# naver/deep-image-retrieval

Measured on AMD Instinct MI355X. Metric: images/sec descriptor extraction (resnet101-GeM, 1024x1024), higher is better.
Workload: dtype fp16p

## Files before the change

### deep-image-retrieval_amd/csrc/c_api.hip

```cpp
#include <new>

#include "engine.h"
#include "pointwise.h"

namespace dir {
const char* last_error();
}
using namespace dir;

static constexpr int kSimSplitMinRows = 32768;

#define DIR_TRY try {
#define DIR_CATCH                                                   \
    }                                                               \
    catch (const std::bad_alloc&) {                                 \
        return fail(DIR_ERR_NOMEM, "out of host memory");           \
    }                                                               \
    catch (const std::exception& ex) {                              \
        return fail(DIR_ERR_INVALID, std::string("exception: ") + ex.what()); \
    }                                                               \
    catch (...) {                                                   \
        return fail(DIR_ERR_INVALID, "unknown exception");          \
    }

// ... 405 lines not shown

static int fill_conv_args(ConvArgs& a, const void* x, const void* w, const float* bias,
                          const void* res, void* y, int B, int H, int W, int Cin, int Cout, int R,
                          int S, int stride, int pad, int OH, int OW, int relu) {
    if (!x || !w || !bias || !y) return fail(DIR_ERR_INVALID, "conv: null pointer");
    if (B <= 0 || H <= 0 || W <= 0 || Cin <= 0 || Cout <= 0 || R <= 0 || S <= 0 || stride <= 0 ||
        pad < 0 || OH <= 0 || OW <= 0)
        return fail(DIR_ERR_INVALID, "conv: bad dimension");
    memset(&a, 0, sizeof(a));
    a.x = (const uint16_t*)x;
    a.w = (const uint16_t*)w;
    a.bias = bias;
    a.res = (const uint16_t*)res;
    a.y = (uint16_t*)y;
    a.B = B; a.H = H; a.W = W; a.Cin = Cin; a.OH = OH; a.OW = OW; a.Cout = Cout;
    a.R = R; a.S = S; a.stride = stride; a.pad = pad; a.relu = relu ? 1 : 0;
    a.M = B * OH * OW;
    a.Ktot = R * S * Cin;
    a.T = a.Ktot / 64;
    return DIR_OK;
}

int dir_conv_bn_act(const void* x, const void* w, const float* bias, const void* res, void* y,
                    int B, int H, int W, int Cin, int Cout, int R, int S, int stride, int pad,
                    int OH, int OW, int relu, int dtype, int variant, void* stream) {
    DIR_TRY
    ConvArgs a;
    int rc = fill_conv_args(a, x, w, bias, res, y, B, H, W, Cin, Cout, R, S, stride, pad, OH, OW, relu);
    if (rc != DIR_OK) return rc;
    return conv_launch(a, dtype, variant, (hipStream_t)stream);
    DIR_CATCH
}

int dir_conv_bn_act_splitk(const void* x, const void* w, const float* bias, const void* res, void* y,
                           int B, int H, int W, int Cin, int Cout, int R, int S, int stride, int pad,
                           int OH, int OW, int relu, int dtype, int variant, int ksplit, void* scratch,
                           size_t scratch_bytes, int* ksplit_used, void* stream) {
    DIR_TRY
    ConvArgs a;
    int rc = fill_conv_args(a, x, w, bias, res, y, B, H, W, Cin, Cout, R, S, stride, pad, OH, OW, relu);
    if (rc != DIR_OK) return rc;
    if (variant < 0) variant = conv_pick_variant(a);
    a.ksplit = ksplit < 0 ? conv_splitk_factor(variant, a) : ksplit;
    a.partial = (float*)scratch;
    if (a.ksplit > 1 && conv_splitk_bytes(a, a.ksplit) > scratch_bytes)
        return fail(DIR_ERR_WORKSPACE, "conv: split-K scratch too small");
    if (ksplit_used) *ksplit_used = a.ksplit > 1 ? a.ksplit : 1;
    return conv_launch(a, dtype, variant, (hipStream_t)stream);
    DIR_CATCH
}

int dir_conv_c3c1(const void* t2, const void* w3, const float* bias3, const void* res, void* y, const void* w1,
                  const float* bias1, void* t1, int B, int H, int W, int P, int P2, int relu3, int relu1, int dtype,
                  void* stream) {
    DIR_TRY
    ConvArgs a;
    int rc = fill_conv_args(a, t2, w3, bias3, res, y, B, H, W, P, 4 * P, 1, 1, 1, 0, H, W, relu3);
    if (rc != DIR_OK) return rc;
    if (!w1 || !bias1 || !t1 || !res) return fail(DIR_ERR_INVALID, "conv_c3c1: null pointer");
    if (dtype != DIR_BF16 && dtype != DIR_FP16) return fail(DIR_ERR_INVALID, "conv_c3c1: bad dtype");
    a.w2 = (const uint16_t*)w1;
    a.bias2 = bias1;
    a.y2 = (uint16_t*)t1;
    a.Cout2 = P2;
    a.relu2 = relu1 ? 1 : 0;
    if (!conv_c3c1_admissible(a))
// ... 344 lines not shown
```

### deep-image-retrieval_amd/csrc/conv_patchw.hip

```cpp
#include "dir_common.h"
#include "conv_igemm.h"

#ifndef DIR_PATCHW_ABL
#define DIR_PATCHW_ABL 0
#endif

namespace dir {

static constexpr uint32_t kOOBw = 0x80000000u;

__device__ __forceinline__ void dma16w(__amdgpu_buffer_rsrc_t rsrc, char* lds, uint32_t voff, int soff) {
    __builtin_amdgcn_raw_ptr_buffer_load_lds(rsrc, (DIR_LDS void*)lds, 16, voff, soff, 0, 0);
}

template <class DT>
__global__ void __launch_bounds__(512) conv_patch3x3w_kernel(const ConvArgs a) {
    constexpr int TH = 16, TW = 32, PH = TH + 2, PW = TW + 2, PP = PH * PW;
    constexpr int NTH = 512, BN = 128;
    constexpr int NPL = (PP * 4 + NTH - 1) / NTH;
    constexpr int PLANE_BYTES = NPL * NTH * 16;
    constexpr int TN = 4, TMR = 2;
    constexpr int WSTAGE = 3 * BN * 64, NBW = WSTAGE / (NTH * 16);
    constexpr int NBW_X = (DIR_PATCHW_ABL & 16) ? 2 : 0;
    constexpr int NPL_X = (DIR_PATCHW_ABL & 32) ? 7 : 0;
    constexpr int NSTW = 3;
    constexpr int WOFF = 2 * PLANE_BYTES;
    constexpr int EROW = TN * 128 + 16;
    typedef typename DT::frag_t frag_t;
    static_assert(WOFF + NSTW * WSTAGE <= 160 * 1024 && NBW * NTH * 16 == WSTAGE, "LDS map");

    extern __shared__ __attribute__((aligned(16))) char smem[];

// ... 378 lines not shown
            const f32x4_t f1 = *(const f32x4_t*)(ebase + mrow * EROW + ecol * 4 + 16);
            const int ox = ox0 + mrow;
            if (oy < a.OH && ox < a.OW) {
                float v[8] = {f0[0], f0[1], f0[2], f0[3], f1[0], f1[1], f1[2], f1[3]};
                const size_t o = ((size_t)(b * a.OH + oy) * a.OW + ox) * a.Cout + ncol;
                if (a.res) {
                    const u32x4_t rv = gload16(a.res + o);
#pragma unroll
                    for (int e = 0; e < 4; ++e) {
                        float lo, hi;
                        DT::unpack(rv[e], lo, hi);
                        v[2 * e] += lo;
                        v[2 * e + 1] += hi;
                    }
                }
                if (a.relu) {
#pragma unroll
                    for (int e = 0; e < 8; ++e) v[e] = fmaxf(v[e], 0.f);
                }
                u32x4_t ov;
#pragma unroll
                for (int e = 0; e < 4; ++e) ov[e] = DT::pack(v[2 * e], v[2 * e + 1]);
                gstore16(a.y + o, ov);
                ovf.see(ov);
            }
        }
        __builtin_amdgcn_fence(__ATOMIC_RELEASE, "wavefront");
        __builtin_amdgcn_wave_barrier();
        __builtin_amdgcn_fence(__ATOMIC_ACQUIRE, "wavefront");
    }
    ovf.flush(a.ovf);
}

bool conv_patch3x3w_admissible(const ConvArgs& a) {
    return a.R == 3 && a.S == 3 && a.stride == 1 && a.pad == 1 && a.H == a.OH && a.W == a.OW && a.Cin % 32 == 0 &&
           a.Cin >= 64 && a.Cout % 128 == 0 && (size_t)a.B * a.H * a.W * a.Cin * 2 < (1ull << 31) &&
           (size_t)a.Cout * a.Ktot * 2 < (1ull << 31);
}

__global__ void __launch_bounds__(256) pack_patchw_kernel(const uint16_t* w, uint16_t* out, int Cout, int Cin) {
    const int NQ = Cin / 32;
    const long pieces = (long)Cout * 9 * Cin / 8;
    for (long i = (long)blockIdx.x * 256 + threadIdx.x; i < pieces; i += (long)gridDim.x * 256) {
        const int L = (int)(i % 1536);
        long t = i / 1536;
        const int r = (int)(t % 3);
        t /= 3;
        const int q = (int)(t % NQ);
        const int tn = (int)(t / NQ);
        const int s = L >> 9, n = (L & 511) >> 2, pos = L & 3;
        const size_t src = ((size_t)((tn * 128 + n) * 9 + r * 3 + s)) * Cin + q * 32 + ((pos ^ ((n >> 2) & 3)) << 3);
        gstore16(out + i * 8, gload16(w + src));
    }
}

hipError_t conv_patch3x3w_pack(const uint16_t* w, uint16_t* out, int Cout, int Cin, hipStream_t stream) {
    const long pieces = (long)Cout * 9 * Cin / 8;
    const int grid = (int)((pieces + 255) / 256 < 1024 ? (pieces + 255) / 256 : 1024);
    hipLaunchKernelGGL(pack_patchw_kernel, dim3(grid), dim3(256), 0, stream, w, out, Cout, Cin);
    return hipGetLastError();
}

template <class DT>
static hipError_t launch_patch_w(const ConvArgs& a, hipStream_t stream) {
    constexpr int LDS = 2 * 5 * 512 * 16 + 3 * 3 * 128 * 64;
    static_assert(LDS <= 160 * 1024 && LDS >= 8 * 32 * (4 * 128 + 16), "LDS map (the staging area aliases it)");
    ConvArgs b = a;
    b.x_bytes = (uint32_t)((size_t)a.B * a.H * a.W * a.Cin * 2);
    b.w_bytes = (uint32_t)((size_t)a.Cout * a.Ktot * 2);
    const long blocks = (long)a.B * ((a.OH + 15) / 16) * ((a.OW + 31) / 32) * (a.Cout / 128);
    if (!env().no_patchw_lc) {
        void* scratch = nullptr;
        if (!b.w_pw && env().patchw_pack) {
            if (hipError_t e = hipMallocAsync(&scratch, b.w_bytes, stream); e != hipSuccess) return e;
            if (hipError_t e = conv_patch3x3w_pack(a.w, (uint16_t*)scratch, a.Cout, a.Cin, stream); e != hipSuccess) {
                (void)hipFreeAsync(scratch, stream);
                return e;
            }
            b.w_pw = (const uint16_t*)scratch;
        }
        auto kern = conv_patch3x3w_lc_kernel<DT>;
        static std::atomic<uint64_t> attr_lc{0};
        if (hipError_t e = ensure_dynamic_lds((const void*)kern, LDS, attr_lc); e != hipSuccess) return e;
        hipLaunchKernelGGL(kern, dim3((unsigned)blocks), dim3(768), LDS, stream, b);
        hipError_t e = hipGetLastError();
        if (scratch) {
            const hipError_t f = hipFreeAsync(scratch, stream);
            if (e == hipSuccess) e = f;
        }
        return e;
    }
    auto kern = conv_patch3x3w_kernel<DT>;
    static std::atomic<uint64_t> attr_done{0};
    if (hipError_t e = ensure_dynamic_lds((const void*)kern, LDS, attr_done); e != hipSuccess) return e;
    hipLaunchKernelGGL(kern, dim3((unsigned)blocks), dim3(512), LDS, stream, b);
    return hipGetLastError();
}

hipError_t conv_patch3x3w_launch(const ConvArgs& a, int dtype, hipStream_t stream) {
    return dtype == DIR_BF16 ? launch_patch_w<BF16>(a, stream) : launch_patch_w<FP16>(a, stream);
}

}
```

### deep-image-retrieval_amd/csrc/dir_common.h

```cpp
#pragma once
#include <hip/hip_runtime.h>
#include <stdint.h>
#include <string.h>
#include <atomic>
#include <string>

#include "../../include/dir_engine.h"

namespace dir {

typedef __attribute__((ext_vector_type(8))) __bf16 bf16x8_t;
typedef __attribute__((ext_vector_type(8))) _Float16 f16x8_t;
typedef __attribute__((ext_vector_type(16))) float f32x16_t;
typedef __attribute__((ext_vector_type(4))) float f32x4_t;
typedef __attribute__((ext_vector_type(4))) uint32_t u32x4_t;
typedef __attribute__((ext_vector_type(2))) uint32_t u32x2_t;
typedef __attribute__((ext_vector_type(2))) float f32x2_t;
typedef __attribute__((ext_vector_type(2))) __bf16 bf16x2_t;
typedef __attribute__((ext_vector_type(2))) _Float16 f16x2_t;

#define DIR_GLOBAL __attribute__((address_space(1)))
#define DIR_LDS __attribute__((address_space(3)))

void set_error(const std::string& msg);
int fail(int code, const std::string& msg);

#define DIR_HIP_CHECK(expr)                                                                \
    do {                                                                                   \
        hipError_t _e = (expr);                                                            \
        if (_e != hipSuccess)                                                              \
            return ::dir::fail(DIR_ERR_HIP, std::string(#expr) + ": " + hipGetErrorString(_e)); \
    } while (0)

struct Env {
    bool c3c1_off = false, c3c1_force = false;
    bool no_ds_seam = false, no_dual = false;
    bool rev_conv1 = false, rev_conv3 = false;
    bool unfused_stem = false, stem_v1 = false;
    bool no_patchlc = false, no_wreg = false, no_patchw = false, no_x3 = false, no_patchs = false;
    bool patchw_pack = false, no_patchw_pack = false;
    bool small_k2 = false;
    bool no_patchs2 = false;
    bool x3_k2048 = false;
    bool lc1x1 = false;
    bool no_c3c1lc = false;
    bool no_smallmap = false;
    bool no_wregd = false;
    bool no_patchw_lc = false;
    bool no_xcdmap = false;
    bool no_pair_patch = false, pair_acts = false;
    int pair_stages = 1;
    bool sim_v1 = false, sim_exact = false;
    bool experiments = false;
    bool no_inplace = false;
    bool no_stem_u8 = false;
    bool stem_pair_old = false;
    bool stem_u8_prep = false;
    bool stem_u8_wg8 = false;
    int stem_u8_seg = 0;
};
const Env& env();
void reload_env();

__host__ __device__ inline uint16_t f32_to_bf16_bits(float f) {
    uint32_t u;
    memcpy(&u, &f, 4);
    if ((u & 0x7fffffffu) > 0x7f800000u) return (uint16_t)((u >> 16) | 0x40);
    u += 0x7fffu + ((u >> 16) & 1u);
    return (uint16_t)(u >> 16);
}
__host__ __device__ inline float bf16_bits_to_f32(uint16_t h) {
    uint32_t u = ((uint32_t)h) << 16;
    float f;
    memcpy(&f, &u, 4);
    return f;
}
__host__ __device__ inline uint16_t f32_to_f16_bits(float f) {
    _Float16 h = (_Float16)f;
    uint16_t b;
    memcpy(&b, &h, 2);
    return b;
// ... 128 lines not shown
```

### deep-image-retrieval_amd/csrc/engine.hip

```cpp
#include "engine.h"

#include <math.h>
#include <algorithm>

namespace dir {

static thread_local std::string g_err;
void set_error(const std::string& msg) { g_err = msg; }
int fail(int code, const std::string& msg) {
    g_err = msg;
    return code;
}
const char* last_error() { return g_err.c_str(); }


static Env read_env() {
    Env e;
    auto on = [](const char* k) { return getenv(k) != nullptr; };
    const char* mode = getenv("DIRTORCH_AMD_C3C1");
    e.c3c1_off = mode && mode[0] == '0';
    e.c3c1_force = mode && mode[0] == 'f';
    e.no_ds_seam = on("DIRTORCH_AMD_NO_DS_SEAM");
    e.no_dual = on("DIRTORCH_AMD_NO_DUAL");
    e.rev_conv1 = on("DIRTORCH_AMD_REV_CONV1");
    e.rev_conv3 = on("DIRTORCH_AMD_REV_CONV3");
    e.unfused_stem = on("DIRTORCH_AMD_UNFUSED_STEM");
    e.stem_v1 = on("DIRTORCH_AMD_STEM_V1");
    e.no_patchlc = on("DIRTORCH_AMD_NO_PATCHLC");
    e.no_wreg = on("DIRTORCH_AMD_NO_WREG");
    e.no_wregd = on("DIRTORCH_AMD_NO_WREGD");
    e.no_smallmap = on("DIRTORCH_AMD_NO_SMALLMAP");
    e.no_c3c1lc = on("DIRTORCH_AMD_NO_C3C1LC");
    e.lc1x1 = on("DIRTORCH_AMD_LC1X1");
    e.x3_k2048 = on("DIRTORCH_AMD_X3_K2048");
    e.no_patchs2 = on("DIRTORCH_AMD_NO_PATCHS2");
    e.small_k2 = on("DIRTORCH_AMD_SMALL_K2");
    e.patchw_pack = on("DIRTORCH_AMD_PATCHW_PACK");
    e.no_patchw_pack = on("DIRTORCH_AMD_NO_PATCHW_PACK");
    e.no_patchw = on("DIRTORCH_AMD_NO_PATCHW");
    e.no_x3 = on("DIRTORCH_AMD_NO_X3");
    e.no_patchs = on("DIRTORCH_AMD_NO_PATCHS");
    e.no_patchw_lc = on("DIRTORCH_AMD_NO_PATCHW_LC");
    e.no_xcdmap = on("DIRTORCH_AMD_NO_XCDMAP");
    e.no_pair_patch = on("DIRTORCH_AMD_NO_PAIR_PATCH");
    e.pair_acts = on("DIRTORCH_AMD_PAIR_ACTS");
    if (const char* s = getenv("DIRTORCH_AMD_PAIR_STAGES")) e.pair_stages = atoi(s);
    e.sim_v1 = on("DIRTORCH_AMD_SIM_V1");
    e.sim_exact = on("DIRTORCH_AMD_SIM_EXACT");
    e.experiments = on("DIRTORCH_AMD_EXPERIMENTS");
    e.no_inplace = on("DIRTORCH_AMD_NO_INPLACE");
    e.no_stem_u8 = on("DIRTORCH_AMD_NO_STEM_U8");
    e.stem_u8_wg8 = on("DIRTORCH_AMD_STEM_U8_WG8");
    e.stem_u8_prep = on("DIRTORCH_AMD_STEM_U8_PREP");
    e.stem_pair_old = on("DIRTORCH_AMD_STEM_PAIR_OLD");
    if (const char* s = getenv("DIRTORCH_AMD_STEM_U8_SEG")) e.stem_u8_seg = atoi(s);
    return e;
}
static Env g_env[2];
static std::atomic<int> g_env_cur{-1};
static std::atomic_flag g_env_lock = ATOMIC_FLAG_INIT;
static void publish_env() {
    while (g_env_lock.test_and_set(std::memory_order_acquire)) {
    }
    const int cur = g_env_cur.load(std::memory_order_relaxed);
    const int nxt = cur < 0 ? 0 : 1 - cur;
    g_env[nxt] = read_env();
    g_env_cur.store(nxt, std::memory_order_release);
    g_env_lock.clear(std::memory_order_release);
}
const Env& env() {
    int cur = g_env_cur.load(std::memory_order_acquire);
    if (cur < 0) {
        static const bool once = (publish_env(), true);
        (void)once;
        cur = g_env_cur.load(std::memory_order_acquire);
// ... 1190 lines not shown
```

### deep-image-retrieval_amd/dirtorch_amd/_lib.py

```python
import ctypes
import os
from ctypes import (POINTER, Structure, c_char, c_char_p, c_double, c_float, c_int, c_int64,
                    c_size_t, c_void_p)

_HERE = os.path.dirname(os.path.abspath(__file__))
LIB_PATH = os.environ.get('DIRTORCH_AMD_LIB') or os.path.join(_HERE, 'libdir_engine.so')

DIR_BF16, DIR_FP16, DIR_F32, DIR_FP16P = 0, 1, 2, 3
DIR_ERR_RANGE = -7
DTYPES = {'bf16': DIR_BF16, 'fp16': DIR_FP16, 'f32': DIR_F32, 'fp16p': DIR_FP16P}
DIR_IMG_F32_NCHW, DIR_IMG_U8_NHWC = 0, 1
DIR_POOL_GEM, DIR_POOL_MAX, DIR_POOL_AVG = 0, 1, 2
POOLING = {'gem': DIR_POOL_GEM, 'max': DIR_POOL_MAX, 'avg': DIR_POOL_AVG}
DIR_HEAD_RMAC, DIR_HEAD_FPN, DIR_HEAD_FPN0, DIR_HEAD_CLASSIFIER = 0, 1, 2, 3


class DirError(RuntimeError):

    def __init__(self, code, msg):
        super().__init__('dir_engine error %d: %s' % (code, msg))
        self.code = code


class ModelDesc(Structure):
# ... 3 lines not shown
                ('head', c_int)]


class ProfRecord(Structure):
    _fields_ = [('name', c_char * 48), ('kernel', c_char * 48), ('flops', c_double),
                ('bytes', c_double), ('ms', c_float)]


SIGNATURES = {
    'dir_last_error': (c_char_p, []),
    'dir_version': (c_char_p, []),
    'dir_engine_create': (c_int, [POINTER(ModelDesc), c_int, POINTER(c_void_p)]),
    'dir_engine_destroy': (c_int, [c_void_p]),
    'dir_engine_set_tensor': (c_int, [c_void_p, c_char_p, c_void_p, POINTER(c_int64), c_int]),
    'dir_engine_finalize': (c_int, [c_void_p, c_int]),
    'dir_engine_out_dim': (c_int, [c_void_p, POINTER(c_int)]),
    'dir_workspace_bytes': (c_int, [c_void_p, c_int, c_int, c_int, POINTER(c_size_t)]),
    'dir_forward': (c_int, [c_void_p, c_void_p, c_int, c_int, c_int, c_int, c_void_p, c_void_p,
                            c_size_t, c_void_p]),
    'dir_forward_features': (c_int, [c_void_p, c_void_p, c_int, c_int, c_int, c_int, c_void_p,
                                     POINTER(c_int), POINTER(c_int), POINTER(c_int), c_void_p,
                                     c_size_t, c_void_p]),
    'dir_engine_autotune': (c_int, [c_void_p, c_int, c_int, c_int, c_void_p, c_size_t, c_void_p]),
    'dir_engine_tuning_export': (c_int, [c_void_p, c_char_p, c_size_t, POINTER(c_size_t)]),
    'dir_engine_tuning_import': (c_int, [c_void_p, c_char_p]),
    'dir_engine_set_profiling': (c_int, [c_void_p, c_int]),
    'dir_engine_profile_pause': (c_int, [c_void_p, c_int]),
    'dir_engine_get_profile': (c_int, [c_void_p, POINTER(ProfRecord), c_int, POINTER(c_int)]),
    'dir_conv_variant_count': (c_int, []),
    'dir_reload_env': (c_int, []),
    'dir_conv_variant_name': (c_int, [c_int, c_char_p, c_int]),
    'dir_conv_bn_act': (c_int, [c_void_p, c_void_p, c_void_p, c_void_p, c_void_p] + [c_int] * 14
                        + [c_void_p]),
    'dir_conv_bn_act_f32': (c_int, [c_void_p, c_void_p, c_void_p, c_void_p, c_void_p] + [c_int] * 12 + [c_void_p]),
    'dir_conv_bn_act_pair': (c_int, [c_void_p] * 4 + [c_void_p] + [c_void_p] * 4 + [c_int] * 12 + [c_void_p]),
    'dir_conv_pair_dual': (c_int, [c_void_p] * 9 + [c_int] * 6 + [c_void_p]),
    'dir_prep_input_pair': (c_int, [c_void_p, c_int, POINTER(c_float), POINTER(c_float), c_void_p, c_void_p,
                                    c_int, c_int, c_int, c_void_p]),
    'dir_stem_pool_pair': (c_int, [c_void_p] * 7 + [c_int] * 5 + [c_void_p]),
    'dir_stem_pool_u8': (c_int, [c_void_p] * 9 + [c_int] * 4 + [c_void_p]),
    'dir_engine_overflow': (c_int, [c_void_p, c_void_p, POINTER(c_int)]),
    'dir_conv_heuristic': (c_int, [c_int] * 12 + [c_char_p, c_int, POINTER(c_int)]),
    'dir_conv_variant_admissible': (c_int, [c_int] * 13 + [POINTER(c_int)]),
    'dir_conv_variant_splitk': (c_int, [c_int] * 13 + [POINTER(c_int)]),
    'dir_conv_bn_act_splitk': (c_int, [c_void_p, c_void_p, c_void_p, c_void_p, c_void_p] + [c_int] * 15 +
                               [c_void_p, c_size_t, POINTER(c_int), c_void_p]),
    'dir_conv_c3c1': (c_int, [c_void_p, c_void_p, c_void_p, c_void_p, c_void_p, c_void_p, c_void_p, c_void_p]
                      + [c_int] * 8 + [c_void_p]),
    'dir_conv_c3c1_ds': (c_int, [c_void_p, c_void_p, c_void_p, c_void_p, c_void_p, c_void_p, c_void_p, c_void_p]
                         + [c_int] * 6 + [c_void_p]),
    'dir_conv_c3c1_wpair': (c_int, [c_void_p] * 10 + [c_int] * 6 + [c_void_p]),
    'dir_conv_c3c1_ds_wpair': (c_int, [c_void_p] * 11 + [c_int] * 5 + [c_void_p]),
    'dir_conv_dual': (c_int, [c_void_p, c_void_p, c_void_p, c_void_p, c_void_p] + [c_int] * 11 + [c_void_p]),
    'dir_conv_bn_act_naive': (c_int, [c_void_p, c_void_p, c_void_p, c_void_p, c_void_p]
                              + [c_int] * 13 + [c_void_p]),
    'dir_prep_input': (c_int, [c_void_p, c_int, POINTER(c_float), POINTER(c_float), c_void_p,
                               c_int, c_int, c_int, c_int, c_void_p]),
    'dir_stem_pool': (c_int, [c_void_p, c_void_p, c_void_p, c_void_p, c_int, c_int, c_int, c_int, c_int,
                              c_int, c_void_p]),
    'dir_maxpool_3x3s2': (c_int, [c_void_p, c_void_p, c_int, c_int, c_int, c_int, c_int, c_void_p]),
    'dir_global_pool': (c_int, [c_void_p, c_void_p, c_int, c_int, c_int, c_int, c_int, c_float,
                                c_float, c_float, c_int, c_void_p]),
    'dir_resize_workspace_bytes': (c_int, [c_int, c_int, c_int, c_int, c_int, POINTER(c_size_t)]),
    'dir_resize_bilinear_u8': (c_int, [c_void_p, c_void_p, c_int, c_int, c_int, c_int, c_int, c_void_p,
                                       c_size_t, c_void_p]),
    'dir_upsample_add': (c_int, [c_void_p, c_void_p, c_void_p, c_int, c_int, c_int, c_int, c_int,
# ... 73 lines not shown
```

### deep-image-retrieval_amd/dirtorch_amd/ops.py

```python
import ctypes

import torch

from . import _lib
from ._lib import DIR_BF16, DIR_FP16, POOLING, call, ptr, stream_ptr


def _dtype_code(t):
    if t.dtype == torch.bfloat16:
        return DIR_BF16
    if t.dtype == torch.float16:
        return DIR_FP16
    raise TypeError('16-bit activation tensor expected (bfloat16 or float16), got %s' % t.dtype)


def _need_cuda(*ts):
    for t in ts:
        if t is not None and not t.is_cuda:
            raise ValueError('device tensor expected')
        if t is not None and not t.is_contiguous():
            raise ValueError('contiguous tensor expected')


def conv_variant_names():
# ... 12 lines not shown

def pack_stem_weight(w_oihw, dtype=torch.bfloat16):
    O = w_oihw.shape[0]
    out = torch.zeros(O, 4, 4, 16, dtype=torch.float32, device=w_oihw.device)
    for R in range(4):
        for S in range(4):
            for dy in range(2):
                for dx in range(2):
                    r, s = 2 * R + dy - 1, 2 * S + dx - 1
                    if 0 <= r < 7 and 0 <= s < 7:
                        c0 = (dy * 2 + dx) * 3
                        out[:, R, S, c0:c0 + 3] = w_oihw[:, :, r, s]
    return out.to(dtype)


def conv_bn_act_f32(x, w, bias, res=None, stride=1, pad=0, relu=True):
    _need_cuda(x, w, bias, res)
    for t in (x, w, bias, res):
        if t is not None and t.dtype != torch.float32:
            raise TypeError('fp32 tensors expected')
    B, H, W, Cin = x.shape
    Cout, R, S, Cin2 = w.shape
    if Cin2 != Cin:
        raise ValueError('Cin mismatch')
    OH = (H + 2 * pad - R) // stride + 1
    OW = (W + 2 * pad - S) // stride + 1
    y = torch.empty(B, OH, OW, Cout, dtype=torch.float32, device=x.device)
    call('dir_conv_bn_act_f32', ptr(x), ptr(w), ptr(bias), ptr(res), ptr(y), B, H, W, Cin, Cout, R, S, stride, pad,
         OH, OW, int(bool(relu)), stream_ptr())
    return y


def conv_bn_act(x, w, bias, res=None, stride=1, pad=0, relu=True, out_hw=None, variant=-1,
                naive=False, ksplit=None):
    _need_cuda(x, w, bias, res)
    B, H, W, Cin = x.shape
    Cout, R, S, Cin2 = w.shape
    if Cin2 != Cin:
        raise ValueError('Cin mismatch')
    if out_hw is None:
        OH = (H + 2 * pad - R) // stride + 1
        OW = (W + 2 * pad - S) // stride + 1
    else:
        OH, OW = out_hw
    y = torch.empty(B, OH, OW, Cout, dtype=x.dtype, device=x.device)
    args = [ptr(x), ptr(w), ptr(bias), ptr(res), ptr(y), B, H, W, Cin, Cout, R, S, stride, pad, OH,
            OW, int(bool(relu)), _dtype_code(x)]
    if ksplit is not None:
        n = max(int(ksplit), 1)
        if ksplit < 0:
            q = ctypes.c_int()
            shape = (B, H, W, Cin, Cout, R, S, stride, pad, OH, OW, int(res is not None))
            if variant < 0:
                call('dir_conv_heuristic', *shape, ctypes.create_string_buffer(64), 64, ctypes.byref(q))
            else:
                call('dir_conv_variant_splitk', int(variant), *shape, ctypes.byref(q))
            n = q.value
        scratch = torch.empty(n * B * OH * OW * Cout if n > 1 else 0, dtype=torch.float32, device=x.device)
        used = ctypes.c_int()
        call('dir_conv_bn_act_splitk', *args, int(variant), int(ksplit), ptr(scratch), scratch.numel() * 4,
             ctypes.byref(used), stream_ptr())
        conv_bn_act.last_ksplit = used.value
    elif naive:
        call('dir_conv_bn_act_naive', *args, stream_ptr())
    else:
        call('dir_conv_bn_act', *args, int(variant), stream_ptr())
    return y


def conv_c3c1(t2, w3, bias3, res, w1, bias1, relu3=True, relu1=True):
    _need_cuda(t2, w3, bias3, res, w1, bias1)
    B, H, W, P = t2.shape
    P2 = w1.shape[0]
    y = torch.empty(B, H, W, 4 * P, dtype=t2.dtype, device=t2.device)
    t1 = torch.empty(B, H, W, P2, dtype=t2.dtype, device=t2.device)
    call('dir_conv_c3c1', ptr(t2), ptr(w3), ptr(bias3), ptr(res), ptr(y), ptr(w1), ptr(bias1), ptr(t1), B, H, W, P, P2,
         int(bool(relu3)), int(bool(relu1)), _dtype_code(t2), stream_ptr())
    return y, t1


def conv_c3c1_ds(t2, x, wcat, bias, w1, bias1, relu3=True, relu1=True):
    _need_cuda(t2, x, wcat, bias, w1, bias1)
    B, H, W, P = t2.shape
    y = torch.empty(B, H, W, 256, dtype=t2.dtype, device=t2.device)
    t1 = torch.empty(B, H, W, 64, dtype=t2.dtype, device=t2.device)
    call('dir_conv_c3c1_ds', ptr(t2), ptr(x), ptr(wcat), ptr(bias), ptr(y), ptr(w1), ptr(bias1), ptr(t1), B, H, W,
         int(bool(relu3)), int(bool(relu1)), _dtype_code(t2), stream_ptr())
    return y, t1


def conv_c3c1_wpair(t2, w3, bias3, res, w1, bias1, relu3=True, relu1=True):
    (w3h, w3l), (w1h, w1l) = w3, w1
    _need_cuda(t2, w3h, w3l, bias3, res, w1h, bias1)
    B, H, W, P = t2.shape
    P2 = w1h.shape[0]
    y = torch.empty(B, H, W, 4 * P, dtype=t2.dtype, device=t2.device)
    t1 = torch.empty(B, H, W, P2, dtype=t2.dtype, device=t2.device)
# ... 299 lines not shown
```

### include/dir_engine.h

```cpp
#ifndef DIR_ENGINE_H
#define DIR_ENGINE_H

#include <stddef.h>
#include <stdint.h>

#ifdef __cplusplus
extern "C" {
#endif

typedef enum dir_status {
    DIR_OK = 0,
    DIR_ERR_INVALID = -1,
    DIR_ERR_STATE = -2,
    DIR_ERR_MISSING = -3,
    DIR_ERR_WORKSPACE = -4,
    DIR_ERR_HIP = -5,
    DIR_ERR_NOMEM = -6,
    DIR_ERR_RANGE = -7
} dir_status;

typedef enum dir_dtype {
    DIR_BF16 = 0,
    DIR_FP16 = 1,
    DIR_F32 = 2,
// ... 58 lines not shown
                         int Cout, int R, int S, int stride, int pad, int OH, int OW, int relu, void* stream);
int dir_conv_pair_dual(const void* t2_hi, const void* t2_lo, const void* x_hi, const void* x_lo, const void* wcat_hi,
                       const void* wcat_lo, const float* bias, void* y_hi, void* y_lo, int B, int H, int W, int Cin,
                       int Cout, int relu, void* stream);
int dir_prep_input_pair(const void* img, int img_format, const float* mean3, const float* std3, void* out_hi,
                        void* out_lo, int B, int H, int W, void* stream);
int dir_stem_pool_pair(const void* s2d_hi, const void* s2d_lo, const void* w_hi, const void* w_lo, const float* bias,
                       void* y_hi, void* y_lo, int B, int H2, int W2, int OH, int OW, void* stream);
int dir_stem_pool_u8(const void* img_u8, const float* w_oihw, const float* bn_scale, const float* bn_bias, const float* mean3,
                     const float* std3, void* s2d_ws, void* y_hi, void* y_lo, int B, int H, int W, int seg_tiles, void* stream);
int dir_engine_overflow(dir_engine* e, void* stream, int* overflowed);

int dir_engine_autotune(dir_engine* e, int B, int H, int W, void* workspace,
                        size_t workspace_bytes, void* stream);
int dir_engine_tuning_export(const dir_engine* e, char* buf, size_t cap, size_t* needed);
int dir_engine_tuning_import(dir_engine* e, const char* text);

typedef struct dir_prof_record {
    char     name[48];
    char     kernel[48];
    double   flops;
    double   bytes;
    float    ms;
} dir_prof_record;
int dir_engine_set_profiling(dir_engine* e, int enabled);
int dir_engine_profile_pause(dir_engine* e, int paused);
int dir_engine_get_profile(dir_engine* e, dir_prof_record* out, int cap, int* n);

int dir_conv_variant_count(void);
int dir_conv_variant_name(int variant, char* buf, int cap);
int dir_conv_bn_act(const void* x, const void* w, const float* bias, const void* res, void* y,
                    int B, int H, int W, int Cin, int Cout, int R, int S, int stride,
                    int pad, int OH, int OW, int relu, int dtype, int variant, void* stream);
int dir_conv_heuristic(int B, int H, int W, int Cin, int Cout, int R, int S, int stride, int pad, int OH,
                       int OW, int has_residual, char* name, int cap, int* ksplit);
int dir_conv_variant_admissible(int variant, int B, int H, int W, int Cin, int Cout, int R, int S, int stride, int pad,
                                int OH, int OW, int has_residual, int* admissible);
int dir_conv_variant_splitk(int variant, int B, int H, int W, int Cin, int Cout, int R, int S, int stride, int pad,
                            int OH, int OW, int has_residual, int* ksplit);
int dir_conv_bn_act_splitk(const void* x, const void* w, const float* bias, const void* res, void* y,
                           int B, int H, int W, int Cin, int Cout, int R, int S, int stride, int pad,
                           int OH, int OW, int relu, int dtype, int variant, int ksplit, void* scratch,
                           size_t scratch_bytes, int* ksplit_used, void* stream);
int dir_conv_c3c1(const void* t2, const void* w3, const float* bias3, const void* res, void* y, const void* w1,
                  const float* bias1, void* t1, int B, int H, int W, int P, int P2, int relu3, int relu1, int dtype,
                  void* stream);
int dir_conv_dual(const void* t2, const void* x, const void* wcat, const float* bias, void* y, int B, int OH, int OW,
                  int Cin, int Cout, int Cin2, int H2, int W2, int stride2, int relu, int dtype, void* stream);
int dir_conv_c3c1_ds(const void* t2, const void* x, const void* wcat, const float* bias, void* y, const void* w1,
                     const float* bias1, void* t1, int B, int H, int W, int relu3, int relu1, int dtype,
                     void* stream);
int dir_conv_c3c1_wpair(const void* t2, const void* w3, const void* w3_lo, const float* bias3, const void* res, void* y,
                        const void* w1, const void* w1_lo, const float* bias1, void* t1, int B, int H, int W, int P2,
                        int relu3, int relu1, void* stream);
int dir_conv_c3c1_ds_wpair(const void* t2, const void* x, const void* x_lo, const void* wcat, const void* wcat_lo,
                           const float* bias, void* y, const void* w1, const void* w1_lo, const float* bias1, void* t1,
                           int B, int H, int W, int relu3, int relu1, void* stream);
int dir_conv_bn_act_naive(const void* x, const void* w, const float* bias, const void* res,
                          void* y, int B, int H, int W, int Cin, int Cout, int R, int S,
                          int stride, int pad, int OH, int OW, int relu, int dtype, void* stream);
int dir_prep_input(const void* img, int img_format, const float* mean3, const float* std3,
                   void* out, int B, int H, int W, int dtype, void* stream);
int dir_stem_pool(const void* s2d, const void* w, const float* bias, void* y, int B, int H2, int W2,
                  int OH, int OW, int dtype, void* stream);
int dir_resize_workspace_bytes(int B, int H, int W, int OH, int OW, size_t* bytes);
int dir_resize_bilinear_u8(const void* src, void* dst, int B, int H, int W, int OH, int OW,
// ... 44 lines not shown
```

Before: 2436.

## Add persistent warp-specialized 3x3 patch conv kernel with cross-tile prefetch

Adds a persistent variant of the 3x3 stride-1 patch conv kernel that launches one block per CU and loops over output tiles. Loader waves prefetch the next tile's input plane and weights, and write back the previous tile's staged outputs while compute waves run, so DMA, epilogue and MFMA work overlap across tiles and the per-block launch and tail costs are spread out. It is picked by default when there are more blocks than CUs, Cin is a multiple of 64 and there is no residual; an environment flag turns it off. A separate conv entry point that takes an overflow word is also exposed; this is new API surface rather than a speed change. The risks are a more complex vmcnt and barrier schedule and less parallelism on small layers.

Result: no change. 2441, median of 6 (+0.2%).

```diff
diff --git a/deep-image-retrieval_amd/csrc/c_api.hip b/deep-image-retrieval_amd/csrc/c_api.hip
--- a/deep-image-retrieval_amd/csrc/c_api.hip
+++ b/deep-image-retrieval_amd/csrc/c_api.hip
@@ -461,6 +461,18 @@
     DIR_CATCH
 }
 
+int dir_conv_bn_act_ovf(const void* x, const void* w, const float* bias, const void* res, void* y,
+                        int B, int H, int W, int Cin, int Cout, int R, int S, int stride, int pad,
+                        int OH, int OW, int relu, int dtype, int variant, int* ovf, void* stream) {
+    DIR_TRY
+    ConvArgs a;
+    int rc = fill_conv_args(a, x, w, bias, res, y, B, H, W, Cin, Cout, R, S, stride, pad, OH, OW, relu);
+    if (rc != DIR_OK) return rc;
+    a.ovf = ovf;
+    return conv_launch(a, dtype, variant, (hipStream_t)stream);
+    DIR_CATCH
+}
+
 int dir_conv_bn_act_splitk(const void* x, const void* w, const float* bias, const void* res, void* y,
                            int B, int H, int W, int Cin, int Cout, int R, int S, int stride, int pad,
                            int OH, int OW, int relu, int dtype, int variant, int ksplit, void* scratch,
diff --git a/deep-image-retrieval_amd/csrc/conv_patchw.hip b/deep-image-retrieval_amd/csrc/conv_patchw.hip
--- a/deep-image-retrieval_amd/csrc/conv_patchw.hip
+++ b/deep-image-retrieval_amd/csrc/conv_patchw.hip
@@ -1,3 +1,5 @@
+#include <type_traits>
+
 #include "dir_common.h"
 #include "conv_igemm.h"
 
@@ -442,6 +444,294 @@
     ovf.flush(a.ovf);
 }
 
+template <class DT>
+__global__ void __launch_bounds__(768) conv_patch3x3w_plc_kernel(const ConvArgs a) {
+    constexpr int TH = 16, TW = 32, PH = TH + 2, PW = TW + 2, PP = PH * PW;
+    constexpr int NLD = 256, BN = 128;
+    constexpr int NPL = (PP * 4 + NLD - 1) / NLD;
+    constexpr int PLANE_BYTES = NPL * NLD * 16;
+    constexpr int TN = 4, TMR = 2;
+    constexpr int WSTAGE = 3 * BN * 64, NBW = WSTAGE / (NLD * 16);
+    constexpr int NSTW = 3;
+    constexpr int W01_OFF = PLANE_BYTES;
+    constexpr int P1_OFF = PLANE_BYTES + 2 * WSTAGE;
+    constexpr int W2_OFF = P1_OFF + PLANE_BYTES;
+    constexpr int STG_OFF = P1_OFF, SROW = BN * 2, NSTH = TH * TW / 2 * SROW / (NLD * 16);
+    constexpr int NSTG = 4;
+    typedef typename DT::frag_t frag_t;
+    static_assert(W2_OFF + WSTAGE <= 160 * 1024 && NBW * NLD * 16 == WSTAGE, "LDS map");
+    static_assert(STG_OFF + TH * TW / 2 * SROW == W2_OFF + WSTAGE && NSTH == 16, "staging = plane buffer 1 + weight slot 2");
+
+    extern __shared__ __attribute__((aligned(16))) char smem[];
+
+    const int tid = threadIdx.x;
+    const int lane = tid & 63;
+    const int wave = __builtin_amdgcn_readfirstlane(tid >> 6);
+    const int lrow = lane & 31, lhi = lane >> 5;
+
+    const int NQ = a.Cin / 32;
+    const int NS = NQ * 3;
+    const int tiles_n = a.Cout / BN;
+    const int tiles_x = (a.OW + TW - 1) / TW;
+    const int tiles_y = (a.OH + TH - 1) / TH;
+    const int total = tiles_n * tiles_x * tiles_y * a.B;
+    const int my_tiles = (total - (int)blockIdx.x + (int)gridDim.x - 1) / (int)gridDim.x;
+    struct Tile {
+        int tile_n, b, oy0, ox0;
+    };
+    auto tile_at = [&](int k) {
+        int wg = xcd_remap((int)blockIdx.x + k * (int)gridDim.x, total);
+        Tile t;
+        t.tile_n = wg % tiles_n;
+        wg /= tiles_n;
+        t.ox0 = (wg % tiles_x) * TW;
+        wg /= tiles_x;
+        t.oy0 = (wg % tiles_y) * TH;
+        t.b = wg / tiles_y;
+        return t;
+    };
+    auto plane_at = [&](int q) { return smem + ((q & 1) ? P1_OFF : 0); };
+    auto slot_at = [&](int slot) { return smem + (slot == 2 ? W2_OFF : W01_OFF + slot * WSTAGE); };
+
+    if (wave >= 8) {
+        const int lt = tid - 512;
+        const int lw = wave - 8;
+        const __amdgpu_buffer_rsrc_t rsrc_x = __builtin_amdgcn_make_buffer_rsrc((void*)a.x, 0, a.x_bytes, 0x00020000);
+        const uint32_t y_bytes = (uint32_t)((size_t)a.B * a.OH * a.OW * a.Cout * 2);
+        const __amdgpu_buffer_rsrc_t rsrc_y = __builtin_amdgcn_make_buffer_rsrc((void*)a.y, 0, y_bytes, 0x00020000);
+        uint32_t pvoff[NPL];
+        auto set_pvoff = [&](const Tile& t) {
+#pragma unroll
+            for (int i = 0; i < NPL; ++i) {
+                const int P = i * NLD + lt;
+                const int p = P >> 2, pos = P & 3;
+                const int py = p / PW, px = p - py * PW;
+                const int iy = t.oy0 - 1 + py, ix = t.ox0 - 1 + px;
+                const bool ok = p < PP && (unsigned)iy < (unsigned)a.H && (unsigned)ix < (unsigned)a.W;
+                pvoff[i] = ok ? (uint32_t)((((t.b * a.H + iy) * a.W + ix) * a.Cin + ((pos ^ ((p >> 2) & 3)) << 3)) * 2) : kOOBw;
+            }
+        };
+        const bool packed = a.w_pw != nullptr;
+        const __amdgpu_buffer_rsrc_t rsrc_wp = __builtin_amdgcn_make_buffer_rsrc((void*)(packed ? a.w_pw : a.w), 0, a.w_bytes, 0x00020000);
+        uint32_t wvoff[NBW];
+#pragma unroll
+        for (int i = 0; i < NBW; ++i) {
+            const int L = i * NLD + lt;
+            const int s = L >> 9, n = (L & 511) >> 2, pos = L & 3;
+            wvoff[i] = packed ? (uint32_t)(L * 16) : (uint32_t)(((n * 9 + s) * a.Cin + ((pos ^ ((n >> 2) & 3)) << 3)) * 2);
+        }
+        auto issue_plane = [&](int q) {
+            char* dst = plane_at(q);
+#pragma unroll
+            for (int i = 0; i < NPL; ++i) dma16w(rsrc_x, dst + (i * NLD + lw * 64) * 16, pvoff[i], q * 64);
+        };
+        auto issue_w = [&](int tile_n, int sigma, int slot) {
+            const int q = sigma / 3, r = sigma - q * 3;
+            char* dst = slot_at(slot);
+            const int soff = packed ? (tile_n * NS + sigma) * WSTAGE : ((tile_n * BN * 9 + r * 3) * a.Cin + q * 32) * 2;
+#pragma unroll
+            for (int i = 0; i < NBW; ++i) dma16w(rsrc_wp, dst + (i * NLD + lw * 64) * 16, wvoff[i], soff);
+        };
+        auto wait_vm = [&](int n) {
+            switch (n) {
+#define DIR_PLC_WAIT(N) case N: asm volatile("s_waitcnt vmcnt(" #N ")" ::: "memory"); break;
+                DIR_PLC_WAIT(4) DIR_PLC_WAIT(6) DIR_PLC_WAIT(10) DIR_PLC_WAIT(14) DIR_PLC_WAIT(16) DIR_PLC_WAIT(22)
+                DIR_PLC_WAIT(24) DIR_PLC_WAIT(36)
+#undef DIR_PLC_WAIT
+                default: asm volatile("s_waitcnt vmcnt(0)" ::: "memory"); break;
+            }
+        };
+        const int spix = lt >> 4, schunk = lt & 15;
+        auto read_half = [&](u32x4_t* h) {
+#pragma unroll
+            for (int k = 0; k < NSTH; ++k) h[k] = *(const u32x4_t*)(smem + STG_OFF + (k * 16 + spix) * SROW + ((schunk ^ spix) << 4));
+            asm volatile("s_waitcnt lgkmcnt(0)" ::: "memory");
+        };
+        auto store_chunk = [&](const u32x4_t v, int k, int j, const Tile& t) {
+            const int oy = t.oy0 + 2 * (k >> 1) + j, ox = t.ox0 + (k & 1) * 16 + spix;
+            const uint32_t off = oy < a.OH && ox < a.OW
+                                     ? ((uint32_t)((t.b * a.OH + oy) * a.OW + ox) * (uint32_t)a.Cout + (uint32_t)(t.tile_n * BN + schunk * 8)) * 2
+                                     : kOOBw;
+            __builtin_amdgcn_raw_buffer_store_b128(v, rsrc_y, off, 0, 0);
+        };
+
+        Tile cur = tile_at(0), done = cur;
+        set_pvoff(cur);
+        issue_plane(0);
+        issue_w(cur.tile_n, 0, 0);
+        issue_w(cur.tile_n, 1, 1);
+        int in_prev = NBW;
+        int st_prev = 0, st_prev2 = 0;
+        bool pend = false;
+        u32x4_t hreg[NSTH];
+        for (int k = 0; k < my_tiles; ++k) {
+            const bool has_next = k + 1 < my_tiles;
+            const Tile nxt = has_next ? tile_at(k + 1) : cur;
+            int q = 0, r = 0, slot_c = 0;
+            for (int sigma = 0; sigma < NS; ++sigma) {
+                wait_vm(st_prev2 + in_prev);
+                ring_barrier();
+                int in_now = 0, st_now = 0;
+                if (r == 0) {
+                    if (q + 1 < NQ) {
+                        issue_plane(q + 1);
+                        in_now += NPL;
+                        if (q + 2 == NQ && has_next) set_pvoff(nxt);
+                    } else if (has_next) {
+                        issue_plane(0);
+                        in_now += NPL;
+                    }
+                }
+                int slot_n = slot_c + 2;
+                if (slot_n >= NSTW) slot_n -= NSTW;
+                if (sigma + 2 < NS) {
+                    issue_w(cur.tile_n, sigma + 2, slot_n);
+                    in_now += NBW;
+                } else if (has_next) {
+                    issue_w(nxt.tile_n, sigma + 2 - NS, slot_n);
+                    in_now += NBW;
+                }
+                if (pend && sigma < NSTG) {
+#pragma unroll
+                    for (int g = 0; g < NSTG; ++g)
+                        if (sigma == g) {
+#pragma unroll
+                            for (int e = 0; e < NSTH / NSTG; ++e) store_chunk(hreg[g * (NSTH / NSTG) + e], g * (NSTH / NSTG) + e, 1, done);
+                        }
+                    in_now += NSTH / NSTG;
+                    st_now = NSTH / NSTG;
+                    if (sigma == NSTG - 1) pend = false;
+                }
+                st_prev2 = st_prev;
+                st_prev = st_now;
+                in_prev = in_now;
+                if (++slot_c == NSTW) slot_c = 0;
+                if (++r == 3) {
+                    r = 0;
+                    ++q;
+                }
+            }
+            ring_barrier();
+            ring_barrier();
+            read_half(hreg);
+            ring_barrier();
+#pragma unroll
+            for (int e = 0; e < NSTH; ++e) store_chunk(hreg[e], e, 0, cur);
+            in_prev += NSTH;
+            st_prev += NSTH;
+            ring_barrier();
+            read_half(hreg);
+            pend = true;
+            done = cur;
+            cur = nxt;
+        }
+#pragma unroll
+        for (int e = 0; e < NSTH; ++e) store_chunk(hreg[e], e, 1, done);
+        return;
+    }
+
+    Tile cur = tile_at(0);
+    f32x16_t acc[TN][TMR];
+#pragma unroll
+    for (int i = 0; i < TN; ++i)
+#pragma unroll
+        for (int g = 0; g < 4; ++g) {
+            const f32x4_t b4 = *(const DIR_GLOBAL f32x4_t*)(a.bias + cur.tile_n * BN + i * 32 + 8 * g + 4 * lhi);
+#pragma unroll
+            for (int j = 0; j < TMR; ++j)
+#pragma unroll
+                for (int e = 0; e < 4; ++e) acc[i][j][4 * g + e] = b4[e];
+        }
+    int woffk[2];
+#pragma unroll
+    for (int kk = 0; kk < 2; ++kk) woffk[kk] = lrow * 64 + (((2 * kk + lhi) ^ ((lrow >> 2) & 3)) << 4);
+    asm volatile("s_waitcnt vmcnt(0)" ::: "memory");
+    char* const swr = smem + STG_OFF + (wave * 32 + lrow) * SROW + lhi * 8;
+    const int sswz = lrow & 15;
+    Ovf<DT> ovf;
+
+    for (int k = 0; k < my_tiles; ++k) {
+        const bool has_next = k + 1 < my_tiles;
+        const Tile nxt = has_next ? tile_at(k + 1) : cur;
+        int q = 0, r = 0, slot_c = 0;
+        for (int sigma = 0; sigma < NS; ++sigma) {
+            ring_barrier();
+            const char* plane = plane_at(q);
+            const char* wst = slot_at(slot_c);
+#pragma unroll
+            for (int s = 0; s < 3; ++s) {
+#pragma unroll
+                for (int kk = 0; kk < 2; ++kk) {
+                    frag_t xf[TMR], wf[TN];
+#pragma unroll
+                    for (int j = 0; j < TMR; ++j) {
+                        const int p = (wave * TMR + j + r) * PW + s + lrow;
+                        xf[j] = *(const frag_t*)(plane + p * 64 + (((2 * kk + lhi) ^ ((p >> 2) & 3)) << 4));
+                    }
+#pragma unroll
+                    for (int i = 0; i < TN; ++i) wf[i] = *(const frag_t*)(wst + s * (BN * 64) + i * 2048 + woffk[kk]);
+#pragma unroll
+                    for (int j = 0; j < TMR; ++j)
+#pragma unroll
+                        for (int i = 0; i < TN; ++i) acc[i][j] = DT::mfma32(wf[i], xf[j], acc[i][j]);
+                }
+            }
+            asm volatile("s_waitcnt lgkmcnt(0)" ::: "memory");
+            if (++slot_c == NSTW) slot_c = 0;
+            if (++r == 3) {
+                r = 0;
+                ++q;
+            }
+        }
+        ring_barrier();
+        int sw = sswz;
+        asm volatile("" : "+v"(sw));
+        auto stage_half = [&](const int j, auto relu) {
+            const uint32_t seen = cur.oy0 + wave * TMR + j < a.OH && cur.ox0 + lrow < a.OW ? 0xffffffffu : 0u;
+#pragma unroll
+            for (int i = 0; i < TN; ++i)
+#pragma unroll
+                for (int g = 0; g < 4; ++g) {
+                    float v[4] = {acc[i][j][4 * g + 0], acc[i][j][4 * g + 1], acc[i][j][4 * g + 2], acc[i][j][4 * g + 3]};
+                    if (decltype(relu)::value) {
+#pragma unroll
+                        for (int e = 0; e < 4; ++e) v[e] = fmaxf(v[e], 0.f);
+                    }
+                    u32x2_t ov;
+                    ov[0] = DT::pack(v[0], v[1]);
+                    ov[1] = DT::pack(v[2], v[3]);
+                    ovf.see(ov[0] & seen);
+                    ovf.see(ov[1] & seen);
+                    *(u32x2_t*)(swr + (((4 * i + g) ^ sw) << 4)) = ov;
+                }
+            asm volatile("s_waitcnt lgkmcnt(0)" ::: "memory");
+        };
+        if (a.relu) stage_half(0, std::true_type{}); else stage_half(0, std::false_type{});
+        ring_barrier();
+        if (has_next) {
+            int bh = 4 * lhi;
+            asm volatile("" : "+v"(bh));
+#pragma unroll
+            for (int i = 0; i < TN; ++i)
+#pragma unroll
+                for (int g = 0; g < 4; ++g) {
+                    const f32x4_t b4 = *(const DIR_GLOBAL f32x4_t*)(a.bias + nxt.tile_n * BN + i * 32 + 8 * g + bh);
+#pragma unroll
+                    for (int e = 0; e < 4; ++e) acc[i][0][4 * g + e] = b4[e];
+                }
+        }
+        ring_barrier();
+        if (a.relu) stage_half(1, std::true_type{}); else stage_half(1, std::false_type{});
+        ring_barrier();
+        if (has_next) {
+#pragma unroll
+            for (int i = 0; i < TN; ++i) acc[i][1] = acc[i][0];
+        }
+        cur = nxt;
+    }
+    ovf.flush(a.ovf);
+}
+
 bool conv_patch3x3w_admissible(const ConvArgs& a) {
     return a.R == 3 && a.S == 3 && a.stride == 1 && a.pad == 1 && a.H == a.OH && a.W == a.OW && a.Cin % 32 == 0 &&
            a.Cin >= 64 && a.Cout % 128 == 0 && (size_t)a.B * a.H * a.W * a.Cin * 2 < (1ull << 31) &&
@@ -489,11 +779,27 @@
             }
             b.w_pw = (const uint16_t*)scratch;
         }
-        auto kern = conv_patch3x3w_lc_kernel<DT>;
-        static std::atomic<uint64_t> attr_lc{0};
-        if (hipError_t e = ensure_dynamic_lds((const void*)kern, LDS, attr_lc); e != hipSuccess) return e;
-        hipLaunchKernelGGL(kern, dim3((unsigned)blocks), dim3(768), LDS, stream, b);
-        hipError_t e = hipGetLastError();
+        const int ncu = cu_count();
+        const bool persist = !env().no_patchw_persist && blocks > ncu && ncu % 8 == 0 && a.Cin % 64 == 0 && !a.res &&
+                             (size_t)a.B * a.OH * a.OW * a.Cout * 2 < (1ull << 31);
+        hipError_t e;
+        if (persist) {
+            auto kern = conv_patch3x3w_plc_kernel<DT>;
+            static std::atomic<uint64_t> attr_plc{0};
+            e = ensure_dynamic_lds((const void*)kern, LDS, attr_plc);
+            if (e == hipSuccess) {
+                hipLaunchKernelGGL(kern, dim3((unsigned)ncu), dim3(768), LDS, stream, b);
+                e = hipGetLastError();
+            }
+        } else {
+            auto kern = conv_patch3x3w_lc_kernel<DT>;
+            static std::atomic<uint64_t> attr_lc{0};
+            e = ensure_dynamic_lds((const void*)kern, LDS, attr_lc);
+            if (e == hipSuccess) {
+                hipLaunchKernelGGL(kern, dim3((unsigned)blocks), dim3(768), LDS, stream, b);
+                e = hipGetLastError();
+            }
+        }
         if (scratch) {
             const hipError_t f = hipFreeAsync(scratch, stream);
             if (e == hipSuccess) e = f;
diff --git a/deep-image-retrieval_amd/csrc/dir_common.h b/deep-image-retrieval_amd/csrc/dir_common.h
--- a/deep-image-retrieval_amd/csrc/dir_common.h
+++ b/deep-image-retrieval_amd/csrc/dir_common.h
@@ -47,6 +47,7 @@
     bool no_smallmap = false;
     bool no_wregd = false;
     bool no_patchw_lc = false;
+    bool no_patchw_persist = false;
     bool no_xcdmap = false;
     bool no_pair_patch = false, pair_acts = false;
     int pair_stages = 1;
diff --git a/deep-image-retrieval_amd/csrc/engine.hip b/deep-image-retrieval_amd/csrc/engine.hip
--- a/deep-image-retrieval_amd/csrc/engine.hip
+++ b/deep-image-retrieval_amd/csrc/engine.hip
@@ -41,6 +41,7 @@
     e.no_x3 = on("DIRTORCH_AMD_NO_X3");
     e.no_patchs = on("DIRTORCH_AMD_NO_PATCHS");
     e.no_patchw_lc = on("DIRTORCH_AMD_NO_PATCHW_LC");
+    e.no_patchw_persist = on("DIRTORCH_AMD_NO_PATCHW_PERSIST");
     e.no_xcdmap = on("DIRTORCH_AMD_NO_XCDMAP");
     e.no_pair_patch = on("DIRTORCH_AMD_NO_PAIR_PATCH");
     e.pair_acts = on("DIRTORCH_AMD_PAIR_ACTS");
diff --git a/deep-image-retrieval_amd/dirtorch_amd/_lib.py b/deep-image-retrieval_amd/dirtorch_amd/_lib.py
--- a/deep-image-retrieval_amd/dirtorch_amd/_lib.py
+++ b/deep-image-retrieval_amd/dirtorch_amd/_lib.py
@@ -59,6 +59,8 @@
     'dir_conv_variant_name': (c_int, [c_int, c_char_p, c_int]),
     'dir_conv_bn_act': (c_int, [c_void_p, c_void_p, c_void_p, c_void_p, c_void_p] + [c_int] * 14
                         + [c_void_p]),
+    'dir_conv_bn_act_ovf': (c_int, [c_void_p, c_void_p, c_void_p, c_void_p, c_void_p] + [c_int] * 14
+                            + [c_void_p, c_void_p]),
     'dir_conv_bn_act_f32': (c_int, [c_void_p, c_void_p, c_void_p, c_void_p, c_void_p] + [c_int] * 12 + [c_void_p]),
     'dir_conv_bn_act_pair': (c_int, [c_void_p] * 4 + [c_void_p] + [c_void_p] * 4 + [c_int] * 12 + [c_void_p]),
     'dir_conv_pair_dual': (c_int, [c_void_p] * 9 + [c_int] * 6 + [c_void_p]),
diff --git a/deep-image-retrieval_amd/dirtorch_amd/ops.py b/deep-image-retrieval_amd/dirtorch_amd/ops.py
--- a/deep-image-retrieval_amd/dirtorch_amd/ops.py
+++ b/deep-image-retrieval_amd/dirtorch_amd/ops.py
@@ -68,7 +68,7 @@
 
 
 def conv_bn_act(x, w, bias, res=None, stride=1, pad=0, relu=True, out_hw=None, variant=-1,
-                naive=False, ksplit=None):
+                naive=False, ksplit=None, ovf=None):
     _need_cuda(x, w, bias, res)
     B, H, W, Cin = x.shape
     Cout, R, S, Cin2 = w.shape
@@ -99,6 +99,10 @@
         conv_bn_act.last_ksplit = used.value
     elif naive:
         call('dir_conv_bn_act_naive', *args, stream_ptr())
+    elif ovf is not None:
+        if ovf.dtype != torch.int32 or not ovf.is_cuda or ovf.numel() != 1:
+            raise ValueError('ovf: one int32 device word expected')
+        call('dir_conv_bn_act_ovf', *args, int(variant), ptr(ovf), stream_ptr())
     else:
         call('dir_conv_bn_act', *args, int(variant), stream_ptr())
     return y
diff --git a/include/dir_engine.h b/include/dir_engine.h
--- a/include/dir_engine.h
+++ b/include/dir_engine.h
@@ -114,6 +114,9 @@
 int dir_conv_bn_act(const void* x, const void* w, const float* bias, const void* res, void* y,
                     int B, int H, int W, int Cin, int Cout, int R, int S, int stride,
                     int pad, int OH, int OW, int relu, int dtype, int variant, void* stream);
+int dir_conv_bn_act_ovf(const void* x, const void* w, const float* bias, const void* res, void* y,
+                        int B, int H, int W, int Cin, int Cout, int R, int S, int stride,
+                        int pad, int OH, int OW, int relu, int dtype, int variant, int* ovf, void* stream);
 int dir_conv_heuristic(int B, int H, int W, int Cin, int Cout, int R, int S, int stride, int pad, int OH,
                        int OW, int has_residual, char* name, int cap, int* ksplit);
 int dir_conv_variant_admissible(int variant, int B, int H, int W, int Cin, int Cout, int R, int S, int stride, int pad,
```
